# Aaron20127/human-3d-reconstruction

Hardware: AMD Instinct MI355X
Metric: images/sec whole-node, DLA-34+SMPL batch-64 512x512; top-k index bit-match (higher is better)
Workload: dtype bf16; 1 GPU; DLA-34+DCNv2 multi_pose + pose/shape heads -> sigmoid/NMS/top-100 decode -> SMPL 6890-vert LBS; 512x512, batch 64 per GPU (BASELINE configs[2]); batch_per_gpu=64, global_batch=64, K=100, smpl_people_per_image=100, parallelism=dp1 (image shards, one all-gather of dets), collective=none (one rank), steps_in_flight=3, hip_graph=False, dcn_margin=auto, images=64 distinct synthetic images (h3d_amd.synth.synth_image_batch, seed 317), weights=synthetic (h3d_amd.synth, seed 0, gain 1.25, offset_scale 0.5)

## Files before the change

### human-3d-reconstruction_amd/_lib.py

```python
import ctypes
import os

_HERE = os.path.dirname(os.path.abspath(__file__))
LIB_PATH = os.path.join(_HERE, "csrc", "libh3d_hip.so")

H3D_F32, H3D_BF16, H3D_F16, H3D_F16X3 = 0, 1, 2, 3
OP_STEM, OP_CONV, OP_DCN, OP_MAXPOOL, OP_UPADD, OP_COPY, OP_HEADS, OP_DCN_V1, OP_DCN_FUSED = 1, 2, 3, 4, 5, 6, 7, 8, 9
OP_CONV_STREAM, OP_DCN_FUSED_F16, OP_DCN_FUSED_STREAM, OP_STEM3, OP_UPDCN_F16 = 10, 11, 12, 13, 14
OP_IM2COL, OP_MAXPOOL3, OP_DEPTH2SPACE = 15, 16, 17
HEADS_MAX = 16
OUT_NHWC, OUT_NCHW_F32, OUT_NHWC_F32, OUT_NHWC_F16 = 0, 1, 2, 3
DCN_INPUT_NHWC, DCN_OUTPUT_NHWC, DCN_F32_MFMA = 1, 2, 4
ABI_VERSION = 4

DCN_AUX_BYTES = 256
DCN_FUSED_BIAS_WMAX, DCN_FUSED_BIAS_AMAX = 32, 34
OPF_DCN_MASK_FINAL, OPF_DCN_RAW_PACK, OPF_DCN_ACT_MAXIMA, TUNE_DCN_ABLATE_MASK = 0x800, 0x100000, 0x200000, 0x1f
OPF_DCN_FUSED_RAW_PACK, OPF_DCN_FUSED_SCALED_INPUT = 0x100000, 0x200000
TUNE_DCN_FUSED_X3_MARGIN2, TUNE_DCN_FUSED_X3_MARGIN6, TUNE_DCN_FUSED_X3_MARGIN4, TUNE_DCN_FUSED_X3_ABLATE_MASK = 0x2000, 0x4000, 0x8000, 0x1f
OPF_DCN_STREAM_NO_SLOTS, OPF_DCN_STREAM_WIDE_MARGIN, OPF_DCN_STREAM_SLOTS512, OPF_DCN_STREAM_F16_INPUT = 0x1000, 0x8000, 0x10000, 0x40000
OPF_DCN_STREAM_STATS, OPF_DCN_STREAM_VARIANT_MASK = 0x20000, 0x58600
TUNE_DCN_STREAM_FORCE_NARROW_WG, TUNE_DCN_STREAM_FORCE_WIDE_WG = 0x200, 0x400
TUNE_DCN_STREAM_F16_DCN5, TUNE_DCN_STREAM_F16_KEEP_DCN3, TUNE_DCN_STREAM_ABLATE_MASK = 0x4000, 0x2000, 0x1f
TUNE_DCN_STREAM_X3_MARGIN2, TUNE_DCN_STREAM_X3_MARGIN3, TUNE_DCN_STREAM_X3_MARGIN4, TUNE_DCN_STREAM_X3_ABLATE_MASK = 0x4000, 0x8000, 0x10000, 0x1f
TUNE_DCN_F16_ONE_WG_PER_CU, TUNE_DCN_F16_ABLATE_MASK = 0x100, 0xff
TUNE_CONV_STREAM_TILE_MASK, TUNE_CONV_STREAM_AUTO, TUNE_CONV_STREAM_ROUND4_RULE, TUNE_CONV_STREAM_ABLATE_MASK = 0xffff, 1, 0x10000000, 0x1f0000
TUNE_CONV_TILE, TUNE_CONV_HALO_TILE, TUNE_CONV_FORCE_GEMM, TUNE_CONV_GEMM_TILE_MASK = 0x1000, 0x2000, 0x4000, 0xf00
TUNE_CONV_X3_TILED, TUNE_CONV_X3_TILE_MASK, TUNE_CONV_X3_CK16, TUNE_CONV_X3_MT2 = 0x1000, 0x1fff, 0x2000, 0x4000
TUNE_UPADD_TAPS_GLOBAL, TUNE_UPADD_TAPS_LDS, OPF_UPADD_FOLDED = 1, 2, 0x100
TUNE_HEADS_SEPARATE_BIAS, TUNE_HEADS_ABLATE_MASK = 0x200, 0xff
TUNE_HEADS_SPARSE_LDS_PATCH, TUNE_HEADS_SPARSE_WAVES4 = 0x400, 0x800


def TUNE_DCN_STREAM_DCN5_XP(xp):
    return xp << 16


def TUNE_DCN_STREAM_DCN5_XP_OF(reserved):
    return (reserved >> 16) & 0xff


def TUNE_CONV_STREAM_TILE(variant, mt, waves):
    return variant << 12 | mt << 8 | waves

# ... 234 lines not shown
```

### human-3d-reconstruction_amd/csrc/conv2.hip

```cpp
#include "common.h"
#include "epilogue.h"

struct Conv2Args {
    const char *in;
    const char *wimg;
    const float *bias;
    const char *res;
    char *out;
    int B, H, W, Cin, in_cs;
    int Ho, Wo, Cout, out_cs, res_cs, relu, out_mode;
    int G, tiles_x, tiles_y;
    int dbg;
    int xcd;
    int f16;
    unsigned long long *stamps;
};

template <int MT, int WAVES, int S = 1, int SLOTS = 2, int NT = 1>
struct Conv2Cfg {
    static constexpr int TH = 2 * WAVES * NT;
    static constexpr int HROWS = (TH - 1) * S + 3;
    static constexpr int HCOLS = 15 * S + 3;
    static constexpr int PPR = S;
    static constexpr int ROWB = PPR * 1024;
    static constexpr int ROWS = HROWS * PPR;
    static constexpr int HALO = ROWS * 1024;
    static constexpr int WROW = 19 * 16;
    static constexpr int WGRP = 32 * WROW;
    static constexpr int WPIECES = (MT * WGRP + 1023) / 1024;
    static constexpr int WALLOC = WPIECES * 1024;
    static constexpr int SLOT = HALO + WALLOC;
    static constexpr int LDS_EPI = WAVES * ((NT * 32 * (64 * MT + 16) + 1023) / 1024 * 1024);
    static constexpr int LDS_RING = SLOTS * SLOT;
    static constexpr int LDS = LDS_RING > LDS_EPI ? LDS_RING : LDS_EPI;
    static constexpr int THREADS = 64 * WAVES;
    static constexpr int HP = (ROWS + WAVES - 1) / WAVES;
    static constexpr int WP = (WPIECES + WAVES - 1) / WAVES;
};

typedef __attribute__((address_space(3))) void lds_void;

template <int MT, int WAVES, int S, int NT>
__device__ __forceinline__ void conv2_issue(const char *in_b, int in_bytes, const char *wimg, int w_bytes, char *base,
                                            const int *hoff, int woff, int wv, int s, int wsrc, int dbg = 0)
{
    using C = Conv2Cfg<MT, WAVES, S, 2, NT>;
    const auto r_in = __builtin_amdgcn_make_buffer_rsrc((void *)in_b, 0, in_bytes, 0x00020000);
    const auto r_w = __builtin_amdgcn_make_buffer_rsrc((void *)wimg, 0, w_bytes, 0x00020000);
#pragma unroll
    for (int j = 0; j < C::HP; ++j) {
        const int p = wv + j * WAVES;
        if (p < C::ROWS && !(dbg & 8)) __builtin_amdgcn_raw_ptr_buffer_load_lds(r_in, (lds_void *)(base + p * 1024), 16, hoff[j], s * 32, 0, 0);
    }
#pragma unroll
    for (int j = 0; j < C::WP; ++j) {
        const int p = wv + j * WAVES;
        if (p < C::WPIECES && !(dbg & 16))
            __builtin_amdgcn_raw_ptr_buffer_load_lds(r_w, (lds_void *)(base + C::HALO + p * 1024), 16, woff, wsrc + p * 1024, 0, 0);
    }
}

template <typename T, int MT, int WAVES, int EPI, int S = 1, int SLOTS = 2, int NT = 1, bool PIPE = false>
__global__ __launch_bounds__(64 * WAVES) void conv2_kernel(Conv2Args a)
{
    using C = Conv2Cfg<MT, WAVES, S, SLOTS, NT>;
    using E = ET<T>;
    static_assert(sizeof(T) == 2, "2-byte element types");
    __shared__ __attribute__((aligned(1024))) char smem[C::LDS];

    const int tid = threadIdx.x;
    const int l = tid & 63, r = l & 31, h = l >> 5;
    const int wv = __builtin_amdgcn_readfirstlane(tid >> 6);
    const int tiles = a.tiles_x * a.tiles_y;
    const int bid = h3d_tile_id(blockIdx.x, gridDim.x, a.xcd);
    const int b = bid / tiles;
    const int t = bid - b * tiles;
    const int ty = t / a.tiles_x, tx = t - ty * a.tiles_x;
    const int oy0 = ty * C::TH, ox0 = tx * 16;
    const int g0 = blockIdx.y * MT;
    const int cout0 = g0 * 32;
    const int nst = a.Cin >> 4;

// ... 12 lines not shown
    }
    const int woff = l * 16;

    const int py = 2 * NT * wv + (r >> 4), px = r & 15;
    const int boff = py * S * C::ROWB + px * S * 48 + h * 16;
    const int aoff = C::HALO + r * C::WROW + h * 16;

    f32x16 acc[MT][NT];
#pragma unroll
    for (int m = 0; m < MT; ++m)
#pragma unroll
        for (int n = 0; n < NT; ++n)
#pragma unroll
            for (int i = 0; i < 16; ++i) acc[m][n][i] = 0.f;

    constexpr int AHEAD = SLOTS > 1 ? SLOTS - 1 : 1;
    constexpr int PMIN = C::ROWS / WAVES + C::WPIECES / WAVES;
    static_assert(AHEAD <= 2 && PMIN <= 63, "counted vmcnt wait");
    constexpr int WAIT_PMIN = 0x0f70 | (PMIN & 15) | ((PMIN >> 4) << 14);
#pragma unroll
    for (int j = 0; j < AHEAD; ++j)
        if (j < nst && (SLOTS > 1 || j == 0))
            conv2_issue<MT, WAVES, S, NT>(in_b, (int)img_bytes, a.wimg, w_bytes, smem + j * C::SLOT, hoff, woff, wv, j, (j * a.G + g0) * C::WGRP, H3D_DBG(a));
    int cslot = 0, pslot = AHEAD % SLOTS;
#ifdef H3D_ABLATE
    unsigned long long t_bar = 0, t_iss = 0;
    const unsigned long long t_start = __builtin_readcyclecounter();
#endif
    for (int s = 0; s < nst; ++s) {
        if constexpr (SLOTS == 1) {
            if (s > 0) {
                __syncthreads();
                conv2_issue<MT, WAVES, S, NT>(in_b, (int)img_bytes, a.wimg, w_bytes, smem, hoff, woff, wv, s, (s * a.G + g0) * C::WGRP, H3D_DBG(a));
            }
        }
        if (AHEAD == 2 && s + 1 < nst) __builtin_amdgcn_s_waitcnt(WAIT_PMIN);
        else __builtin_amdgcn_s_waitcnt(0x0f70);
#ifdef H3D_ABLATE
        const unsigned long long tb0 = __builtin_readcyclecounter();
#endif
        h3d_barrier_keep_vmcnt();
#ifdef H3D_ABLATE
        const unsigned long long tb1 = __builtin_readcyclecounter();
        t_bar += tb1 - tb0;
#endif
        if (SLOTS > 1 && s + AHEAD < nst && !(H3D_DBG(a) & 1))
            conv2_issue<MT, WAVES, S, NT>(in_b, (int)img_bytes, a.wimg, w_bytes, smem + pslot * C::SLOT, hoff, woff, wv, s + AHEAD, ((s + AHEAD) * a.G + g0) * C::WGRP, H3D_DBG(a));
#ifdef H3D_ABLATE
        t_iss += __builtin_readcyclecounter() - tb1;
#endif
        const char *sl = smem + cslot * C::SLOT;
        cslot = cslot + 1 == SLOTS ? 0 : cslot + 1;
        pslot = pslot + 1 == SLOTS ? 0 : pslot + 1;
        if (H3D_DBG(a) & 2) continue;
        if constexpr (PIPE) {
            typename E::frag fb[2][NT], fa[2][MT];
            auto rd = [&](int tap, int q) {
                const int dy = tap / 3, dx = tap - 3 * dy;
#pragma unroll
                for (int n = 0; n < NT; ++n) fb[q][n] = E::lds_frag(sl + boff + (2 * n * S + dy) * C::ROWB + dx * 48);
#pragma unroll
                for (int m = 0; m < MT; ++m) fa[q][m] = E::lds_frag(sl + aoff + m * C::WGRP + tap * 32);
            };
            rd(0, 0);
            __builtin_amdgcn_sched_group_barrier(0x100, MT + NT, 0);
#pragma unroll
            for (int tap = 0; tap < 9; ++tap) {
                if (tap + 1 < 9) rd(tap + 1, (tap + 1) & 1);
#pragma unroll
                for (int m = 0; m < MT; ++m)
#pragma unroll
                    for (int n = 0; n < NT; ++n) E::mma(acc[m][n], fa[tap & 1][m], fb[tap & 1][n]);
                if (tap + 1 < 9) __builtin_amdgcn_sched_group_barrier(0x100, MT + NT, 0);
                __builtin_amdgcn_sched_group_barrier(0x008, MT * NT, 0);
            }
        } else {
#pragma unroll
        for (int tap = 0; tap < 9; ++tap) {
            const int dy = tap / 3, dx = tap - 3 * dy;
            typename E::frag fb[NT];
#pragma unroll
            for (int n = 0; n < NT; ++n) fb[n] = E::lds_frag(sl + boff + (2 * n * S + dy) * C::ROWB + dx * 48);
            typename E::frag fa[MT];
#pragma unroll
            for (int m = 0; m < MT; ++m) fa[m] = E::lds_frag(sl + aoff + m * C::WGRP + tap * 32);
#pragma unroll
            for (int m = 0; m < MT; ++m)
#pragma unroll
                for (int n = 0; n < NT; ++n) E::mma(acc[m][n], fa[m], fb[n]);
        }
        }
    }

#ifdef H3D_ABLATE
    if (a.stamps && blockIdx.x < 65536 && blockIdx.y == 0 && l == 0) {
        const unsigned long long t_loop = __builtin_readcyclecounter() - t_start;
        if (wv < 4) a.stamps[blockIdx.x * H3D_NSTAMP + wv] = t_bar;
        if (wv >= WAVES - 3) a.stamps[blockIdx.x * H3D_NSTAMP + 4 + (wv - (WAVES - 3))] = t_bar;
        if (wv == 0) a.stamps[blockIdx.x * H3D_NSTAMP + 7] = (t_iss << 32) | (t_loop & 0xffffffffull);
    }
#endif
    EpiArgs e;
    e.bias = a.bias; e.res = a.res; e.out = a.out; e.Ho = a.Ho; e.Wo = a.Wo; e.Cout = a.Cout;
    e.out_cs = a.out_cs; e.res_cs = a.res_cs; e.relu = a.relu; e.out_mode = a.out_mode;
    if constexpr (EPI == 2) {
        __syncthreads();
        tile_epilogue_lds<T, MT, NT>(acc, e, b, oy0, ox0, cout0, wv, l, smem + wv * epi_lds_stride<MT, NT>());
    } else {
        tile_epilogue<T, MT, NT, EPI == 1>(acc, e, b, oy0, ox0, cout0, wv, r, h);
    }
}

template <int MT, int WAVES, int S = 1, int SLOTS = 2, int NT = 1, bool PIPE = false>
static int launch_conv2_cfg(const Conv2Args &a0, hipStream_t st)
{
    using C = Conv2Cfg<MT, WAVES, S, SLOTS, NT>;
    static_assert(C::LDS <= 160 * 1024, "LDS budget");
    Conv2Args a = a0;
    a.tiles_x = cdiv(a.Wo, 16);
    a.tiles_y = cdiv(a.Ho, C::TH);
    a.xcd = h3d_xcd_mode();
#ifdef H3D_ABLATE
    a.stamps = h3d_stamp_buffer();
#else
    a.stamps = nullptr;
#endif
    dim3 grid(a.B * a.tiles_x * a.tiles_y, cdiv(cdiv(a.Cout, 32), MT));
    const bool lean = a.out_mode == H3D_OUT_NHWC && a.Cout % 4 == 0 && ((uintptr_t)a.bias & 15) == 0;
    const int epi = (MT >= 2 && lean && a.Cout % 8 == 0 && a.out_cs % 8 == 0 && ((uintptr_t)a.out & 15) == 0 && !(a.dbg & 4)) ? 2 : lean ? 1 : 0;
    return h3d_by_values([&](auto f16, auto e) {
        using T = std::conditional_t<f16, f16_t, bf16_t>;
        constexpr bool pipe = PIPE && e == 2;
        return h3d_launch({"conv2_kernel", h3d_tag<T>{}, MT, WAVES, e, S, SLOTS, NT, h3d_opt(pipe)},
                          conv2_kernel<T, MT, WAVES, e, S, SLOTS, NT, pipe>, grid, dim3(C::THREADS), 0, st, a);
    }, h3d_vals<false, true>{}, a.f16 != 0, h3d_vals<0, 1, 2>{}, epi);
}

int h3d_launch_conv_stream(const h3d_op &op, hipStream_t st)
{
    if (!op.in || !op.w || !op.bias || !op.out) H3D_FAIL(H3D_ERR_ARG, "conv_stream: null pointer");
    if (op.dtype != H3D_BF16 && op.dtype != H3D_F16) H3D_FAIL(H3D_ERR_DTYPE, "conv_stream: bf16 / fp16 plans only (dtype %d)", op.dtype);
    if (op.ksize != 3 || (op.stride != 1 && op.stride != 2) || op.Ho != (op.H - 1) / op.stride + 1 || op.Wo != (op.W - 1) / op.stride + 1)
        H3D_FAIL(H3D_ERR_UNSUPPORTED, "conv_stream: covers 3x3 p1 with stride 1 or 2 (k=%d s=%d, %dx%d -> %dx%d)", op.ksize, op.stride,
                 op.H, op.W, op.Ho, op.Wo);
    if (op.Cin % 16 || op.in_cs % 8 || op.Cin > op.in_cs)
        H3D_FAIL(H3D_ERR_SHAPE, "conv_stream: Cin=%d (stride %d) must be a multiple of 16", op.Cin, op.in_cs);
    if ((size_t)op.H * op.W * op.in_cs * 2 >= 0x7ffffff0ull) H3D_FAIL(H3D_ERR_SHAPE, "conv_stream: image of 2 GiB or more");
    if (op.wrows % 128 || op.wrows < op.Cout)
        H3D_FAIL(H3D_ERR_SHAPE, "conv_stream: packed weight/bias rows %d for Cout %d (Cout padded to 128 expected)", op.wrows, op.Cout);
    if (op.out_mode != H3D_OUT_NCHW_F32 && (op.out_cs % 4 || op.Cout > op.out_cs))
        H3D_FAIL(H3D_ERR_SHAPE, "conv_stream: out channel stride %d", op.out_cs);
    if (op.in2 && (op.in2_cs % 4 || op.Cout > op.in2_cs)) H3D_FAIL(H3D_ERR_SHAPE, "conv_stream: residual stride %d", op.in2_cs);
    Conv2Args a;
    a.in = (const char *)op.in; a.wimg = (const char *)op.w; a.bias = op.bias; a.res = (const char *)op.in2;
    a.out = (char *)op.out; a.B = op.B; a.H = op.H; a.W = op.W; a.Cin = op.Cin; a.in_cs = op.in_cs;
    a.Ho = op.Ho; a.Wo = op.Wo; a.Cout = op.Cout; a.out_cs = op.out_cs; a.res_cs = op.in2_cs; a.relu = op.relu; a.out_mode = op.out_mode;
    a.G = op.wrows / 32; a.tiles_x = a.tiles_y = 0;
    a.f16 = op.dtype == H3D_F16;
    a.dbg = H3D_TUNE_CONV_STREAM_ABLATE_OF(op.reserved);
    const int tile = op.reserved & H3D_TUNE_CONV_STREAM_TILE_MASK;
    const int gq = cdiv(op.Cout, 32);
    auto nblk = [&](int th, int mt) { return (long)op.B * cdiv(op.Wo, 16) * cdiv(op.Ho, th) * cdiv(gq, mt); };
    if (op.stride == 2) {
        switch (tile) {
        case H3D_TUNE_CONV_STREAM_TILE(4, 4, 4): return launch_conv2_cfg<4, 4, 2, 1>(a, st);
        case H3D_TUNE_CONV_STREAM_TILE(4, 4, 8): return launch_conv2_cfg<4, 8, 2, 1>(a, st);
        case H3D_TUNE_CONV_STREAM_TILE(4, 2, 4): return launch_conv2_cfg<2, 4, 2, 1>(a, st);
        default: break;
        }
        if (gq >= 4) return tile == H3D_TUNE_CONV_STREAM_TILE(2, 4, 4) ? launch_conv2_cfg<4, 4, 2>(a, st) : launch_conv2_cfg<4, 4, 2, 1>(a, st);
        if (gq >= 2) return launch_conv2_cfg<2, 4, 2>(a, st);
        return launch_conv2_cfg<1, 4, 2>(a, st);
    }
    if (tile) {
// ... 43 lines not shown
```

### human-3d-reconstruction_amd/csrc/ops.hip

```cpp
#include "common.h"
#include <stdlib.h>

static thread_local char g_err[512] = "";

void h3d_set_error(const char *fmt, ...)
{
    va_list ap;
    va_start(ap, fmt);
    vsnprintf(g_err, sizeof(g_err), fmt, ap);
    va_end(ap);
}

static thread_local char g_kname[160] = "";
static thread_local bool g_dry = false;

bool h3d_note_kernel(const char *fmt, ...)
{
    va_list ap;
    va_start(ap, fmt);
    vsnprintf(g_kname, sizeof(g_kname), fmt, ap);
    va_end(ap);
    return g_dry;
}

// ... 26 lines not shown
#ifdef H3D_ABLATE
    f |= H3D_BUILD_ABLATE;
#endif
    return f;
}

int h3d_launch_conv(const h3d_op &op, hipStream_t st);
int h3d_launch_stem(const h3d_op &op, hipStream_t st);
int h3d_launch_elementwise(const h3d_op &op, hipStream_t st);
int h3d_launch_dcn(const h3d_op &op, hipStream_t st);
int h3d_launch_heads(const h3d_op &op, hipStream_t st);
int h3d_launch_dcn2(const h3d_op &op, hipStream_t st);
int h3d_launch_dcn3(const h3d_op &op, hipStream_t st);
int h3d_launch_dcn3_fold(const h3d_op &op, const h3d_op &up, hipStream_t st, bool *folded);
int h3d_launch_conv_stream(const h3d_op &op, hipStream_t st);
int h3d_launch_dcn4(const h3d_op &op, hipStream_t st);
int h3d_launch_updcn(const h3d_op &op, hipStream_t st);
int h3d_launch_stem3(const h3d_op &op, hipStream_t st);
int h3d_launch_extra(const h3d_op &op, hipStream_t st);

static int run_one(const h3d_op &op, int i, hipStream_t st, const h3d_op *up = nullptr, bool *folded = nullptr);

static int run_at(const h3d_op *ops, int i, int n, hipStream_t st, bool *folded)
{
    *folded = false;
    if (i + 1 < n && ops[i].kind == H3D_OP_DCN_FUSED_STREAM && ops[i + 1].kind == H3D_OP_UPADD && (ops[i + 1].reserved & H3D_OPF_UPADD_FOLDED) &&
        ops[i].out && ops[i + 1].in2 == ops[i].out)
        return run_one(ops[i], i, st, &ops[i + 1], folded);
    return run_one(ops[i], i, st);
}

extern "C" int h3d_op_kernel_name(const h3d_op *op, char *buf, int buflen)
{
    if (!op || !buf || buflen <= 0) H3D_FAIL(H3D_ERR_ARG, "op_kernel_name: null argument");
    g_dry = true;
    g_kname[0] = 0;
    const int rc = run_one(*op, 0, nullptr);
    g_dry = false;
    snprintf(buf, buflen, "%s", g_kname);
    return rc;
}

extern "C" int h3d_run_ops_timed(const h3d_op *ops, int n, void *stream, float *ms)
{
    if (!ops || n <= 0 || !ms) H3D_FAIL(H3D_ERR_ARG, "run_ops_timed: null argument");
    hipStream_t st = (hipStream_t)stream;
    hipEvent_t *ev = (hipEvent_t *)malloc(sizeof(hipEvent_t) * (n + 1));
    if (!ev) H3D_FAIL(H3D_ERR_ARG, "run_ops_timed: out of host memory");
    for (int i = 0; i <= n; ++i) (void)hipEventCreate(&ev[i]);
    int rc = H3D_OK;
    (void)hipEventRecord(ev[0], st);
    for (int i = 0; i < n; ++i) ms[i] = 0.f;
    for (int i = 0; i < n && rc == H3D_OK; ++i) {
        bool folded = false;
        rc = run_at(ops, i, n, st, &folded);
        (void)hipEventRecord(ev[i + 1], st);
        if (folded) {
            ++i;
            ms[i] = -1.f;
            (void)hipEventRecord(ev[i + 1], st);
        }
    }
    if (rc == H3D_OK) {
        (void)hipEventSynchronize(ev[n]);
        for (int i = 0; i < n; ++i) {
            if (ms[i] < 0.f) ms[i] = 0.f;
            else (void)hipEventElapsedTime(&ms[i], ev[i], ev[i + 1]);
        }
    }
    for (int i = 0; i <= n; ++i) (void)hipEventDestroy(ev[i]);
    free(ev);
    return rc;
}

extern "C" int h3d_run_ops(const h3d_op *ops, int n, void *stream)
{
    if (!ops || n < 0) H3D_FAIL(H3D_ERR_ARG, "run_ops: null plan");
    hipStream_t st = (hipStream_t)stream;
    for (int i = 0; i < n; ++i) {
        bool folded = false;
        const int rc = run_at(ops, i, n, st, &folded);
        if (rc != H3D_OK) return rc;
        if (folded) ++i;
    }
    return H3D_OK;
}

static int run_one(const h3d_op &op, int i, hipStream_t st, const h3d_op *up, bool *folded)
{
    int rc;
    if (op.B <= 0 || op.H <= 0 || op.W <= 0 || op.Ho <= 0 || op.Wo <= 0 || op.Cin <= 0 || op.Cout <= 0) {
        h3d_set_error("op %d (kind %d): non-positive dimension", i, op.kind);
        return H3D_ERR_SHAPE;
    }
    switch (op.kind) {
    case H3D_OP_STEM: rc = h3d_launch_stem(op, st); break;
    case H3D_OP_STEM3: rc = h3d_launch_stem3(op, st); break;
    case H3D_OP_CONV: rc = h3d_launch_conv(op, st); break;
// ... 9 lines not shown
    case H3D_OP_UPDCN_F16:
        h3d_set_error("op %d (kind %d): a superseded kernel generation, built only by `make EXTRA=1` (csrc/Makefile)", i, op.kind);
        return H3D_ERR_UNSUPPORTED;
#endif
    case H3D_OP_DCN_FUSED:
    case H3D_OP_DCN_FUSED_STREAM: rc = up ? h3d_launch_dcn3_fold(op, *up, st, folded) : h3d_launch_dcn3(op, st); break;
    case H3D_OP_HEADS: rc = h3d_launch_heads(op, st); break;
    case H3D_OP_MAXPOOL:
    case H3D_OP_UPADD:
    case H3D_OP_COPY: rc = h3d_launch_elementwise(op, st); break;
    case H3D_OP_IM2COL:
    case H3D_OP_MAXPOOL3:
    case H3D_OP_DEPTH2SPACE: rc = h3d_launch_extra(op, st); break;
    default: h3d_set_error("op %d: unknown kind %d", i, op.kind); return H3D_ERR_ARG;
    }
    if (rc != H3D_OK) {
        char tmp[400];
        snprintf(tmp, sizeof(tmp), "%s", h3d_last_error());
        h3d_set_error("op %d (kind %d): %s", i, op.kind, tmp);
    }
    return rc;
}
```

### human-3d-reconstruction_amd/detector.py

```python
import torch

from . import _lib, decode, smpl as _smpl
from .model import create_model
from .utils import _transpose_and_gather_feat

MULTI_POSE_HEADS = {"hm": 1, "wh": 2, "hps": 34, "reg": 2, "hm_hp": 17, "hp_offset": 2}
CTDET_HEADS = {"hm": 80, "wh": 2, "reg": 2}
SMPL_HEADS = {"pose": 72, "shape": 10}
WHOLE_MAP_HEADS = ("hm", "hm_hp", "hp_offset")
PEAK_HEADS = ("hp_offset",)


class LazyHeads(dict):

    def __init__(self, maps, completer):
        super().__init__(maps)
        self._completer = completer

    @property
    def complete(self):
        return self._completer is None

    def rearm(self, completer):
        self._completer = completer
# ... 84 lines not shown
        if opt.task != "multi_pose":
            raise ValueError("task not defined!")
        self.opt = opt
        self.device = torch.device(device)
        self.model = create_model(opt.arch, opt.heads, opt.head_conv, opt.not_use_dcn, dtype=opt.dtype)
        if state_dict is not None:
            self.model.load_state_dict(state_dict, strict=True)
        self.model.to(self.device).eval()
        self.smpl_model = smpl_model
        self.fused_tail = True
        self.sparse_heads = True
        if opt.arch.replace("-", "_") in ("dla_34", "dla34") and opt.dtype in ("bf16", "f16"):
            self.model.engine_flags["split_heads"] = tuple(h for h in opt.heads if h in WHOLE_MAP_HEADS)
            self.model.engine_flags["peak_heads"] = tuple(h for h in opt.heads if h in PEAK_HEADS)
            self.model.engine_flags["fold_upadd"] = True
        if opt.smpl and smpl_model is None:
            self.smpl_model = _smpl.SMPLModel.synthetic()

    @torch.no_grad()
    def run(self, images, meta=None, slot=0, graph=False):
        if graph and meta is None:
            return self._run_graph(images, slot)
        opt = self.opt
        plan = None
        if self.sparse_heads and not opt.flip_test and images.is_cuda and not self.model.training:
            plan = self.model.engine(images.device).forward_eager(images, slot)
        if plan is not None:
            out = plan.outputs
            top = decode._multi_pose_topk(out["hm"], out.get("hm_hp") if opt.hm_hp else None, opt.K, logits=True)
            if plan.sparse_masks[1] and top["hm_inds"] is not None:
# ... 219 lines not shown
```

### human-3d-reconstruction_amd/plan.py

```python
import ctypes

import torch

from . import _lib, arch, arch_hg, arch_res
from ._lib import H3dOp
from .weights import _TORCH_DT, LOWP

_H3D_DT = {"bf16": _lib.H3D_BF16, "f16": _lib.H3D_F16, "f32": _lib.H3D_F32, "f16x3": _lib.H3D_F16X3}
DCN_F16IN = _lib.OPF_DCN_STREAM_F16_INPUT


class View:
    __slots__ = ("buf", "H", "W", "C", "cs", "coff", "es")

    def __init__(self, buf, H, W, C, cs, coff, es):
        self.buf, self.H, self.W, self.C, self.cs, self.coff, self.es = buf, H, W, C, cs, coff, es

    @property
    def ptr(self):
        return self.buf.data_ptr() + self.coff * self.es

    def slice(self, c0, c):
        assert c0 + c <= self.C
        return View(self.buf, self.H, self.W, c, self.cs, self.coff + c0, self.es)
# ... 15 lines not shown
        fuse_upnode_min_f=2,
        dcn_slots512=0,
        dcn_wide_margin=0,
        node_f16=True,
        share_pool=True,
        fuse_stem=True,
        fuse_stem_proj=False,
        mixed_heads=0,
        wide_heads_m2=0,
        x3_dcn_patches=True,
        stem_s2_direct=True,
        conv1x1_th16_min_cin=0,
        lower_heads=True,
        split_heads=(),
        fold_upadd=False,
        peak_heads=(),
    )

    def __init__(self, pw, B, H, W, **flags):
        unknown = set(flags) - set(self.FLAGS)
        if unknown:
            raise TypeError("unknown lowering flags: %s" % sorted(unknown))
        for k, v in self.FLAGS.items():
            setattr(self, k, flags.get(k, v))
        self.stream_s2_min_cin = 64
        if pw.arch == "hourglass" and (H % 128 or W % 128):
            raise RuntimeError("Hourglass-104: input height/width must be multiples of 128 (got %dx%d): the published test "
                               "code pads to (x|127)+1" % (H, W))
        if H % 32 or W % 32:
            raise RuntimeError("input height/width must be multiples of 32 (got %dx%d): the reference pads "
# ... 38 lines not shown
        op.kind, op.dtype, op.B = kind, _H3D_DT[self.dtype], self.B
        if x is not None:
            op.in_, op.H, op.W, op.Cin, op.in_cs = x.ptr, x.H, x.W, x.C, x.cs
        if out is not None:
            op.out, op.Ho, op.Wo, op.Cout, op.out_cs = out.ptr, out.H, out.W, out.C, out.cs
        if x2 is not None:
            op.in2, op.in2_cs = x2.ptr, x2.cs
        for k, v in kw.items():
            setattr(op, k, v)
        if not emit:
            return op
        self.ops.append(op)
        return len(self.ops) - 1

    def conv(self, x, wkey, out=None, bkey=None, bn=None, stride=1, relu=True, res=None, out_mode=_lib.OUT_NHWC,
             pad_cout_to=None):
        wshape = self.pw.sd[wkey].shape
        if (self.stream_convs and self.pw.dtype in LOWP and wshape[2] == 3 and wshape[1] % 16 == 0
                and (stride == 1 or (stride == 2 and wshape[1] >= self.stream_s2_min_cin and self.stream_s2))
                and out_mode == _lib.OUT_NHWC and pad_cout_to is None):
            return self._conv_stream(x, wkey, out, bkey, bn, relu, res, stride)
        wp, bp, cout, cin, k, rows = self.pw.conv(wkey, bkey, bn, pad_cout_to)
        assert cin == x.C, (wkey, cin, x.C)
        Ho = (x.H + 2 * (k // 2) - k) // stride + 1
        Wo = (x.W + 2 * (k // 2) - k) // stride + 1
        if out_mode == _lib.OUT_NHWC_F32:
            out = self._alloc(Ho, Wo, cout, torch.float32)
        elif out is None:
            out = self._alloc(Ho, Wo, cout)
        assert (out.H, out.W, out.C) == (Ho, Wo, cout), (wkey, out.H, out.W, out.C, Ho, Wo, cout)
        tune = 0
        if (k == 1 and stride == 1 and self.conv1x1_th16_min_cin and cin >= self.conv1x1_th16_min_cin and cin % 64 == 0
                and cout > 32 and self.pw.dtype in LOWP):
            tune = _lib.TUNE_CONV_1X1_TILE(4 if cout > 64 else 2, 16)
        self._op(_lib.OP_CONV, x, out, res, w=wp.data_ptr(), bias=bp.data_ptr(), ksize=k, stride=stride, relu=int(relu),
                 out_mode=out_mode, wrows=rows, reserved=tune, wexp=self.pw.wexp.get(wp.data_ptr(), 0))
        return out

    def _conv_stream(self, x, wkey, out, bkey, bn, relu, res, stride=1):
        wimg, bp, cout, cin, rows = self.pw.conv_stream(wkey, bkey, bn)
        assert cin == x.C, (wkey, cin, x.C)
        Ho, Wo = (x.H - 1) // stride + 1, (x.W - 1) // stride + 1
        if out is None:
            out = self._alloc(Ho, Wo, cout)
        assert (out.H, out.W, out.C) == (Ho, Wo, cout), (wkey, out.H, out.W, out.C)
        self._op(_lib.OP_CONV_STREAM, x, out, res, w=wimg.data_ptr(), bias=bp.data_ptr(), ksize=3, stride=stride, relu=int(relu),
                 out_mode=_lib.OUT_NHWC, wrows=rows)
        return out

    def dcn(self, x, om, wkey, bkey, bn):
        wp, bp, cout, cin, k, rows = self.pw.conv(wkey, bkey, bn, as_half=True)
        assert cin == x.C and k == 3
        out = self._alloc(x.H, x.W, cout)
        self._op(_lib.OP_DCN, x, out, om, w=wp.data_ptr(), bias=bp.data_ptr(), ksize=3, stride=1, relu=1, out_mode=_lib.OUT_NHWC,
                 wrows=rows)
        return out

    def pool(self, x, out=None):
        if out is None:
            out = self._alloc(x.H // 2, x.W // 2, x.C)
        assert out.C == x.C
        self._op(_lib.OP_MAXPOOL, x, out, ksize=2, stride=2)
        return out

    def upadd(self, x, skip, wkey, f16=False, private_skip=False):
        w, k = self.pw.up(wkey)
        f = k // 2
        out = self._alloc(x.H * f, x.W * f, x.C)
        assert (skip.H, skip.W, skip.C) == (out.H, out.W, out.C), wkey
        fold = (private_skip and self.ops and self.ops[-1].kind == _lib.OP_DCN_FUSED_STREAM and self.ops[-1].out == skip.ptr
                and (skip.coff, skip.cs) == (0, skip.C))
        self._op(_lib.OP_UPADD, x, out, skip, w=w.data_ptr(), ksize=k, stride=f, out_mode=_lib.OUT_NHWC_F16 if f16 else _lib.OUT_NHWC,
                 reserved=_lib.OPF_UPADD_FOLDED if fold else 0)
        return out

    def _block(self, x, p, stride, residual, out):
        t = self.conv(x, p + ".conv1.weight", bn=p + ".bn1", stride=stride)
        return self.conv(t, p + ".conv2.weight", bn=p + ".bn2", res=residual, out=out)

    def _tree1(self, x, p, cin, cout, stride, level_root, out, cat=None, bottom=None, residual=None):
        Ho, Wo = x.H // stride, x.W // stride
        if cat is None:
            cat = self._alloc(Ho, Wo, 2 * cout + (cin if level_root else 0))
        s_x2, s_x1 = cat.slice(0, cout), cat.slice(cout, cout)
        if residual is not None:
            assert stride > 1 and not level_root and cin != cout and (residual.H, residual.W, residual.C) == (Ho, Wo, cout)
        elif bottom is not None:
            assert stride > 1 and not level_root and (bottom.H, bottom.W, bottom.C) == (Ho, Wo, cin)
        elif stride > 1:
            bottom = self.pool(x, cat.slice(2 * cout, cin) if level_root else None)
        else:
            bottom = x
        if residual is not None:
            pass
        elif cin != cout:
            residual = self.conv(bottom, p + ".project.0.weight", bn=p + ".project.1", relu=False)
        else:
            residual = bottom
        self._block(x, p + ".tree1", stride, residual, s_x1)
        self._block(s_x1, p + ".tree2", 1, s_x1, s_x2)
        return self.conv(cat, p + ".root.conv.weight", bn=p + ".root.bn", out=out)

    def _tree2(self, x, p, cin, cout, out):
        Ho, Wo = x.H // 2, x.W // 2
        cat = self._alloc(Ho, Wo, 2 * cout + cin + cout)
        pooled = self.pool(x, cat.slice(2 * cout, cin))
        x1 = self._tree1(x, p + ".tree1", cin, cout, 2, False, cat.slice(2 * cout + cin, cout),
                         bottom=pooled if self.share_pool else None)
        return self._tree1(x1, p + ".tree2", cout, cout, 1, False, out, cat=cat)

    def _dcn_f16_ok(self, p):
        w = self.pw.sd[p + ".conv.weight"]
        return (self.pw.use_dcn and self.fuse_offsets and self.stream_dcn and self.pw.dtype == "bf16"
                and w.shape[1] == 64 and w.shape[0] <= 64)

    def _node_f16_ok(self, p):
# ... 297 lines not shown
```

### include/h3d.h

```cpp
#ifndef H3D_H
#define H3D_H

#include <stddef.h>
#include <stdint.h>

#ifdef __cplusplus
extern "C" {
#endif

#define H3D_OK 0
#define H3D_ERR_SHAPE (-1)
#define H3D_ERR_DTYPE (-2)
#define H3D_ERR_LAUNCH (-3)
#define H3D_ERR_UNSUPPORTED (-4)
#define H3D_ERR_ARG (-5)

#define H3D_F32 0
#define H3D_BF16 1
#define H3D_F16 2
#define H3D_F16X3 3

const char *h3d_last_error(void);
int h3d_abi_version(void);
#define H3D_ABI_VERSION 4
// ... 196 lines not shown
#define H3D_TUNE_CONV_X3_TILE(mt, waves, th) (H3D_TUNE_CONV_X3_TILED | (mt) << 8 | (waves) << 4 | (th) >> 3)
enum {
    H3D_TUNE_CONV_X3_TILED = 0x1000,
    H3D_TUNE_CONV_X3_TILE_MASK = 0x1fff,
    H3D_TUNE_CONV_X3_CK16 = 0x2000,
    H3D_TUNE_CONV_X3_MT2 = 0x4000
};

enum {
    H3D_TUNE_UPADD_TAPS_GLOBAL = 1,
    H3D_TUNE_UPADD_TAPS_LDS = 2,
    H3D_OPF_UPADD_FOLDED = 0x100
};

enum {
    H3D_TUNE_HEADS_SEPARATE_BIAS = 0x200,
    H3D_TUNE_HEADS_SPARSE_LDS_PATCH = 0x400,
    H3D_TUNE_HEADS_SPARSE_WAVES4 = 0x800,
    H3D_TUNE_HEADS_ABLATE_MASK = 0xff
};

int h3d_dcn_fused_ck(int Cin, int Cout);

int h3d_dcn_far_samples(const h3d_op *op, int32_t *per_tile, void *stream);

int h3d_run_ops(const h3d_op *ops, int n, void *stream);

int h3d_run_ops_timed(const h3d_op *ops, int n, void *stream, float *ms);
int h3d_op_kernel_name(const h3d_op *op, char *buf, int buflen);

// ... 247 lines not shown
```

Baseline: 10820 images/s.

## Fuse tree-entry maxpool and 1x1 projection into stride-2 streamed conv kernel

At DLA tree entries, the 2x2 maxpool, the 1x1 project conv and the stride-2 3x3 conv1 all read the same input. This change folds all three into one streamed conv kernel. The pool is computed from the centre taps already loaded into the halo, and the projection is a second MFMA accumulator fed by projection filters staged in LDS. The plan flags the triple of ops and the runner dispatches the fused launch. This removes two launches and the extra global reads and writes of the pooled tensor. In exchange the kernel uses more LDS and registers, is forced to one slot, and routes some narrow-Cin stride-2 convs through the stream path.

```diff
diff --git a/human-3d-reconstruction_amd/_lib.py b/human-3d-reconstruction_amd/_lib.py
--- a/human-3d-reconstruction_amd/_lib.py
+++ b/human-3d-reconstruction_amd/_lib.py
@@ -28,6 +28,7 @@
 TUNE_CONV_TILE, TUNE_CONV_HALO_TILE, TUNE_CONV_FORCE_GEMM, TUNE_CONV_GEMM_TILE_MASK = 0x1000, 0x2000, 0x4000, 0xf00
 TUNE_CONV_X3_TILED, TUNE_CONV_X3_TILE_MASK, TUNE_CONV_X3_CK16, TUNE_CONV_X3_MT2 = 0x1000, 0x1fff, 0x2000, 0x4000
 TUNE_UPADD_TAPS_GLOBAL, TUNE_UPADD_TAPS_LDS, OPF_UPADD_FOLDED = 1, 2, 0x100
+OPF_TREE_ENTRY, OPF_TREE_ENTRY_PRIVATE_POOL = 0x20000000, 0x40000000
 TUNE_HEADS_SEPARATE_BIAS, TUNE_HEADS_ABLATE_MASK = 0x200, 0xff
 TUNE_HEADS_SPARSE_LDS_PATCH, TUNE_HEADS_SPARSE_WAVES4 = 0x400, 0x800
 
diff --git a/human-3d-reconstruction_amd/csrc/conv2.hip b/human-3d-reconstruction_amd/csrc/conv2.hip
--- a/human-3d-reconstruction_amd/csrc/conv2.hip
+++ b/human-3d-reconstruction_amd/csrc/conv2.hip
@@ -13,10 +13,15 @@
     int dbg;
     int xcd;
     int f16;
+    const char *pw;
+    const float *pbias;
+    char *pout;
+    char *pool_out;
+    int pwrows, pout_cs, pool_cs;
     unsigned long long *stamps;
 };
 
-template <int MT, int WAVES, int S = 1, int SLOTS = 2, int NT = 1>
+template <int MT, int WAVES, int S = 1, int SLOTS = 2, int NT = 1, bool ENTRY = false>
 struct Conv2Cfg {
     static constexpr int TH = 2 * WAVES * NT;
     static constexpr int HROWS = (TH - 1) * S + 3;
@@ -29,7 +34,8 @@
     static constexpr int WGRP = 32 * WROW;
     static constexpr int WPIECES = (MT * WGRP + 1023) / 1024;
     static constexpr int WALLOC = WPIECES * 1024;
-    static constexpr int SLOT = HALO + WALLOC;
+    static constexpr int PALLOC = ENTRY ? MT * 1024 : 0;
+    static constexpr int SLOT = HALO + WALLOC + PALLOC;
     static constexpr int LDS_EPI = WAVES * ((NT * 32 * (64 * MT + 16) + 1023) / 1024 * 1024);
     static constexpr int LDS_RING = SLOTS * SLOT;
     static constexpr int LDS = LDS_RING > LDS_EPI ? LDS_RING : LDS_EPI;
@@ -60,12 +66,22 @@
     }
 }
 
-template <typename T, int MT, int WAVES, int EPI, int S = 1, int SLOTS = 2, int NT = 1, bool PIPE = false>
-__global__ __launch_bounds__(64 * WAVES) void conv2_kernel(Conv2Args a)
-{
-    using C = Conv2Cfg<MT, WAVES, S, SLOTS, NT>;
+template <int MT, int WAVES>
+__device__ __forceinline__ void conv2_issue_proj(const char *pw, int pw_bytes, char *base, int poff, int wv, int s, int mstep)
+{
+    const auto r_p = __builtin_amdgcn_make_buffer_rsrc((void *)pw, 0, pw_bytes, 0x00020000);
+#pragma unroll
+    for (int m = 0; m < MT; ++m)
+        if (m % WAVES == wv) __builtin_amdgcn_raw_ptr_buffer_load_lds(r_p, (lds_void *)(base + m * 1024), 16, poff, m * mstep + s * 32, 0, 0);
+}
+
+template <typename T, int MT, int WAVES, int EPI, int S = 1, int SLOTS = 2, int NT = 1, bool PIPE = false, bool ENTRY = false>
+__global__ __launch_bounds__(64 * WAVES, ENTRY ? 2 : 1) void conv2_kernel(Conv2Args a)
+{
+    using C = Conv2Cfg<MT, WAVES, S, SLOTS, NT, ENTRY>;
     using E = ET<T>;
     static_assert(sizeof(T) == 2, "2-byte element types");
+    static_assert(!ENTRY || (S == 2 && NT == 1 && EPI == 2 && !PIPE && SLOTS == 1 && MT <= WAVES), "ENTRY: the one-slot stride-2 tiles with the LDS-transposed epilogue");
     __shared__ __attribute__((aligned(1024))) char smem[C::LDS];
 
     const int tid = threadIdx.x;
@@ -108,6 +124,20 @@
 #pragma unroll
             for (int i = 0; i < 16; ++i) acc[m][n][i] = 0.f;
 
+    [[maybe_unused]] f32x16 acc2[ENTRY ? MT : 1][1];
+    [[maybe_unused]] const int poff = ((cout0 + (l >> 1)) * a.Cin + (l & 1) * 8) * 2;
+    [[maybe_unused]] const int pw_bytes = a.pwrows * a.Cin * 2;
+    if constexpr (ENTRY) {
+#pragma unroll
+        for (int m = 0; m < MT; ++m)
+#pragma unroll
+            for (int i = 0; i < 16; ++i) acc2[m][0][i] = 0.f;
+    }
+    auto issue = [&](char *base, int s) {
+        conv2_issue<MT, WAVES, S, NT>(in_b, (int)img_bytes, a.wimg, w_bytes, base, hoff, woff, wv, s, (s * a.G + g0) * C::WGRP, H3D_DBG(a));
+        if constexpr (ENTRY) conv2_issue_proj<MT, WAVES>(a.pw, pw_bytes, base + C::HALO + C::WALLOC, poff, wv, s, 32 * a.Cin * 2);
+    };
+
     constexpr int AHEAD = SLOTS > 1 ? SLOTS - 1 : 1;
     constexpr int PMIN = C::ROWS / WAVES + C::WPIECES / WAVES;
     static_assert(AHEAD <= 2 && PMIN <= 63, "counted vmcnt wait");
@@ -115,7 +145,7 @@
 #pragma unroll
     for (int j = 0; j < AHEAD; ++j)
         if (j < nst && (SLOTS > 1 || j == 0))
-            conv2_issue<MT, WAVES, S, NT>(in_b, (int)img_bytes, a.wimg, w_bytes, smem + j * C::SLOT, hoff, woff, wv, j, (j * a.G + g0) * C::WGRP, H3D_DBG(a));
+            issue(smem + j * C::SLOT, j);
     int cslot = 0, pslot = AHEAD % SLOTS;
 #ifdef H3D_ABLATE
     unsigned long long t_bar = 0, t_iss = 0;
@@ -125,7 +155,7 @@
         if constexpr (SLOTS == 1) {
             if (s > 0) {
                 __syncthreads();
-                conv2_issue<MT, WAVES, S, NT>(in_b, (int)img_bytes, a.wimg, w_bytes, smem, hoff, woff, wv, s, (s * a.G + g0) * C::WGRP, H3D_DBG(a));
+                issue(smem, s);
             }
         }
         if (AHEAD == 2 && s + 1 < nst) __builtin_amdgcn_s_waitcnt(WAIT_PMIN);
@@ -139,7 +169,7 @@
         t_bar += tb1 - tb0;
 #endif
         if (SLOTS > 1 && s + AHEAD < nst && !(H3D_DBG(a) & 1))
-            conv2_issue<MT, WAVES, S, NT>(in_b, (int)img_bytes, a.wimg, w_bytes, smem + pslot * C::SLOT, hoff, woff, wv, s + AHEAD, ((s + AHEAD) * a.G + g0) * C::WGRP, H3D_DBG(a));
+            issue(smem + pslot * C::SLOT, s + AHEAD);
 #ifdef H3D_ABLATE
         t_iss += __builtin_readcyclecounter() - tb1;
 #endif
@@ -169,6 +199,7 @@
                 __builtin_amdgcn_sched_group_barrier(0x008, MT * NT, 0);
             }
         } else {
+        [[maybe_unused]] float pm[8];
 #pragma unroll
         for (int tap = 0; tap < 9; ++tap) {
             const int dy = tap / 3, dx = tap - 3 * dy;
@@ -182,6 +213,25 @@
             for (int m = 0; m < MT; ++m)
 #pragma unroll
                 for (int n = 0; n < NT; ++n) E::mma(acc[m][n], fa[m], fb[n]);
+            if constexpr (ENTRY) {
+                if (tap == 4) {
+                    unpack16<T>(fb[0].v, pm);
+                } else if (tap == 5 || tap == 7 || tap == 8) {
+                    float x[8];
+                    unpack16<T>(fb[0].v, x);
+#pragma unroll
+                    for (int k = 0; k < 8; ++k) pm[k] = fmaxf(pm[k], x[k]);
+                }
+            }
+        }
+        if constexpr (ENTRY) {
+            typename E::frag pb;
+            pb.v = pack16<T>(pm);
+#pragma unroll
+            for (int m = 0; m < MT; ++m) E::mma(acc2[m][0], E::lds_frag(sl + C::HALO + C::WALLOC + m * 1024 + r * 32 + h * 16), pb);
+            const int oy = oy0 + py, ox = ox0 + px;
+            if (a.pool_out && blockIdx.y == 0 && oy < a.Ho && ox < a.Wo)
+                *reinterpret_cast<u32x4 *>(a.pool_out + ((((size_t)b * a.Ho + oy) * a.Wo + ox) * a.pool_cs + 16 * s + 8 * h) * 2) = pb.v;
         }
         }
     }
@@ -200,6 +250,10 @@
     if constexpr (EPI == 2) {
         __syncthreads();
         tile_epilogue_lds<T, MT, NT>(acc, e, b, oy0, ox0, cout0, wv, l, smem + wv * epi_lds_stride<MT, NT>());
+        if constexpr (ENTRY) {
+            e.bias = a.pbias; e.res = nullptr; e.out = a.pout; e.out_cs = a.pout_cs; e.res_cs = 0; e.relu = 0;
+            tile_epilogue_lds<T, MT, 1>(acc2, e, b, oy0, ox0, cout0, wv, l, smem + wv * epi_lds_stride<MT, NT>());
+        }
     } else {
         tile_epilogue<T, MT, NT, EPI == 1>(acc, e, b, oy0, ox0, cout0, wv, r, h);
     }
@@ -230,7 +284,26 @@
     }, h3d_vals<false, true>{}, a.f16 != 0, h3d_vals<0, 1, 2>{}, epi);
 }
 
-int h3d_launch_conv_stream(const h3d_op &op, hipStream_t st)
+template <int MT>
+static int launch_conv2_entry(const Conv2Args &a0, hipStream_t st)
+{
+    constexpr int WAVES = 4, S = 2, SLOTS = 1;
+    using C = Conv2Cfg<MT, WAVES, S, SLOTS, 1, true>;
+    static_assert(2 * C::LDS <= 160 * 1024, "LDS budget: two workgroups per CU, as without the project filters");
+    Conv2Args a = a0;
+    a.tiles_x = cdiv(a.Wo, 16);
+    a.tiles_y = cdiv(a.Ho, C::TH);
+    a.xcd = h3d_xcd_mode();
+    a.stamps = nullptr;
+    dim3 grid(a.B * a.tiles_x * a.tiles_y, cdiv(cdiv(a.Cout, 32), MT));
+    return h3d_by_values([&](auto f16) {
+        using T = std::conditional_t<f16, f16_t, bf16_t>;
+        return h3d_launch({"conv2_kernel", h3d_tag<T>{}, MT, WAVES, 2, S, SLOTS, 1, false, true},
+                          conv2_kernel<T, MT, WAVES, 2, S, SLOTS, 1, false, true>, grid, dim3(C::THREADS), 0, st, a);
+    }, h3d_vals<false, true>{}, a.f16 != 0);
+}
+
+static int conv_stream_check(const h3d_op &op)
 {
     if (!op.in || !op.w || !op.bias || !op.out) H3D_FAIL(H3D_ERR_ARG, "conv_stream: null pointer");
     if (op.dtype != H3D_BF16 && op.dtype != H3D_F16) H3D_FAIL(H3D_ERR_DTYPE, "conv_stream: bf16 / fp16 plans only (dtype %d)", op.dtype);
@@ -245,6 +318,11 @@
     if (op.out_mode != H3D_OUT_NCHW_F32 && (op.out_cs % 4 || op.Cout > op.out_cs))
         H3D_FAIL(H3D_ERR_SHAPE, "conv_stream: out channel stride %d", op.out_cs);
     if (op.in2 && (op.in2_cs % 4 || op.Cout > op.in2_cs)) H3D_FAIL(H3D_ERR_SHAPE, "conv_stream: residual stride %d", op.in2_cs);
+    return H3D_OK;
+}
+
+static Conv2Args conv_stream_args(const h3d_op &op)
+{
     Conv2Args a;
     a.in = (const char *)op.in; a.wimg = (const char *)op.w; a.bias = op.bias; a.res = (const char *)op.in2;
     a.out = (char *)op.out; a.B = op.B; a.H = op.H; a.W = op.W; a.Cin = op.Cin; a.in_cs = op.in_cs;
@@ -252,6 +330,49 @@
     a.G = op.wrows / 32; a.tiles_x = a.tiles_y = 0;
     a.f16 = op.dtype == H3D_F16;
     a.dbg = H3D_TUNE_CONV_STREAM_ABLATE_OF(op.reserved);
+    a.pw = nullptr; a.pbias = nullptr; a.pout = nullptr; a.pool_out = nullptr; a.pwrows = a.pout_cs = a.pool_cs = 0;
+    return a;
+}
+
+bool h3d_conv_stream_entry_takes(const h3d_op &pool, const h3d_op &proj, const h3d_op &conv)
+{
+    if (pool.kind != H3D_OP_MAXPOOL || proj.kind != H3D_OP_CONV || conv.kind != H3D_OP_CONV_STREAM) return false;
+    if (!(pool.reserved & H3D_OPF_TREE_ENTRY) || !(proj.reserved & H3D_OPF_TREE_ENTRY) || !(conv.reserved & H3D_OPF_TREE_ENTRY)) return false;
+    const int gq = cdiv(conv.Cout, 32);
+    if ((conv.reserved & ~H3D_OPF_TREE_ENTRY) != (gq >= 4 ? 0 : H3D_TUNE_CONV_STREAM_TILE(4, 2, 4))) return false;
+    if ((proj.reserved & ~H3D_OPF_TREE_ENTRY) || (pool.reserved & ~(H3D_OPF_TREE_ENTRY | H3D_OPF_TREE_ENTRY_PRIVATE_POOL))) return false;
+    if ((conv.dtype != H3D_BF16 && conv.dtype != H3D_F16) || pool.dtype != conv.dtype || proj.dtype != conv.dtype) return false;
+    if (!pool.in || !pool.out || !proj.w || !proj.bias || !proj.out || proj.in2) return false;
+    if (proj.in != pool.out || proj.in_cs != pool.out_cs || conv.in != pool.in || conv.in_cs != pool.in_cs) return false;
+    const int B = conv.B, H = conv.H, W = conv.W, C = conv.Cin;
+    if (B <= 0 || H <= 0 || W <= 0 || C <= 0 || conv.Cout <= 0) return false;
+    if (pool.B != B || proj.B != B || pool.H != H || pool.W != W || (H & 1) || (W & 1)) return false;
+    if (pool.Cin != C || pool.Cout != C || proj.Cin != C || C > pool.out_cs) return false;
+    const int Ho = H / 2, Wo = W / 2;
+    if (conv.ksize != 3 || conv.stride != 2 || conv.Ho != Ho || conv.Wo != Wo || pool.Ho != Ho || pool.Wo != Wo) return false;
+    if (proj.ksize != 1 || proj.stride != 1 || proj.H != Ho || proj.W != Wo || proj.Ho != Ho || proj.Wo != Wo) return false;
+    if (proj.Cout != conv.Cout || proj.relu || proj.wexp || proj.out_mode != H3D_OUT_NHWC || conv.out_mode != H3D_OUT_NHWC) return false;
+    if (conv.Cout % 8 || gq < 2 || proj.wrows < cdiv(conv.Cout, 128) * 128 || (long long)proj.wrows * C * 2 >= 0x7ffffff0ll) return false;
+    if (conv.out_cs % 8 || proj.out_cs % 8 || proj.Cout > proj.out_cs || pool.out_cs % 8) return false;
+    if (((uintptr_t)conv.out & 15) || ((uintptr_t)conv.bias & 15) || ((uintptr_t)proj.out & 15) || ((uintptr_t)proj.bias & 15) || ((uintptr_t)proj.w & 15) ||
+        ((uintptr_t)pool.out & 15))
+        return false;
+    return conv_stream_check(conv) == H3D_OK;
+}
+
+int h3d_launch_conv_stream_entry(const h3d_op &pool, const h3d_op &proj, const h3d_op &conv, hipStream_t st)
+{
+    Conv2Args a = conv_stream_args(conv);
+    a.pw = (const char *)proj.w; a.pbias = proj.bias; a.pout = (char *)proj.out; a.pwrows = proj.wrows; a.pout_cs = proj.out_cs;
+    a.pool_out = (pool.reserved & H3D_OPF_TREE_ENTRY_PRIVATE_POOL) ? nullptr : (char *)pool.out;
+    a.pool_cs = pool.out_cs;
+    return cdiv(conv.Cout, 32) >= 4 ? launch_conv2_entry<4>(a, st) : launch_conv2_entry<2>(a, st);
+}
+
+int h3d_launch_conv_stream(const h3d_op &op, hipStream_t st)
+{
+    H3D_TRY(conv_stream_check(op));
+    const Conv2Args a = conv_stream_args(op);
     const int tile = op.reserved & H3D_TUNE_CONV_STREAM_TILE_MASK;
     const int gq = cdiv(op.Cout, 32);
     auto nblk = [&](int th, int mt) { return (long)op.B * cdiv(op.Wo, 16) * cdiv(op.Ho, th) * cdiv(gq, mt); };
diff --git a/human-3d-reconstruction_amd/csrc/ops.hip b/human-3d-reconstruction_amd/csrc/ops.hip
--- a/human-3d-reconstruction_amd/csrc/ops.hip
+++ b/human-3d-reconstruction_amd/csrc/ops.hip
@@ -64,19 +64,31 @@
 int h3d_launch_dcn3(const h3d_op &op, hipStream_t st);
 int h3d_launch_dcn3_fold(const h3d_op &op, const h3d_op &up, hipStream_t st, bool *folded);
 int h3d_launch_conv_stream(const h3d_op &op, hipStream_t st);
+bool h3d_conv_stream_entry_takes(const h3d_op &pool, const h3d_op &proj, const h3d_op &conv);
+int h3d_launch_conv_stream_entry(const h3d_op &pool, const h3d_op &proj, const h3d_op &conv, hipStream_t st);
 int h3d_launch_dcn4(const h3d_op &op, hipStream_t st);
 int h3d_launch_updcn(const h3d_op &op, hipStream_t st);
 int h3d_launch_stem3(const h3d_op &op, hipStream_t st);
 int h3d_launch_extra(const h3d_op &op, hipStream_t st);
 
 static int run_one(const h3d_op &op, int i, hipStream_t st, const h3d_op *up = nullptr, bool *folded = nullptr);
+static int fail_at(int rc, const h3d_op &op, int i);
 
-static int run_at(const h3d_op *ops, int i, int n, hipStream_t st, bool *folded)
+static int run_at(const h3d_op *ops, int i, int n, hipStream_t st, int *folded)
 {
-    *folded = false;
+    *folded = 0;
     if (i + 1 < n && ops[i].kind == H3D_OP_DCN_FUSED_STREAM && ops[i + 1].kind == H3D_OP_UPADD && (ops[i + 1].reserved & H3D_OPF_UPADD_FOLDED) &&
-        ops[i].out && ops[i + 1].in2 == ops[i].out)
-        return run_one(ops[i], i, st, &ops[i + 1], folded);
+        ops[i].out && ops[i + 1].in2 == ops[i].out) {
+        bool pair = false;
+        const int rc = run_one(ops[i], i, st, &ops[i + 1], &pair);
+        *folded = pair;
+        return rc;
+    }
+    if (i + 2 < n && ops[i].kind == H3D_OP_MAXPOOL && (ops[i].reserved & H3D_OPF_TREE_ENTRY) &&
+        h3d_conv_stream_entry_takes(ops[i], ops[i + 1], ops[i + 2])) {
+        *folded = 2;
+        return fail_at(h3d_launch_conv_stream_entry(ops[i], ops[i + 1], ops[i + 2], st), ops[i], i);
+    }
     return run_one(ops[i], i, st);
 }
 
@@ -102,10 +114,10 @@
     (void)hipEventRecord(ev[0], st);
     for (int i = 0; i < n; ++i) ms[i] = 0.f;
     for (int i = 0; i < n && rc == H3D_OK; ++i) {
-        bool folded = false;
+        int folded = 0;
         rc = run_at(ops, i, n, st, &folded);
         (void)hipEventRecord(ev[i + 1], st);
-        if (folded) {
+        for (; folded > 0; --folded) {
             ++i;
             ms[i] = -1.f;
             (void)hipEventRecord(ev[i + 1], st);
@@ -128,10 +140,10 @@
     if (!ops || n < 0) H3D_FAIL(H3D_ERR_ARG, "run_ops: null plan");
     hipStream_t st = (hipStream_t)stream;
     for (int i = 0; i < n; ++i) {
-        bool folded = false;
+        int folded = 0;
         const int rc = run_at(ops, i, n, st, &folded);
         if (rc != H3D_OK) return rc;
-        if (folded) ++i;
+        i += folded;
     }
     return H3D_OK;
 }
@@ -171,6 +183,11 @@
     case H3D_OP_DEPTH2SPACE: rc = h3d_launch_extra(op, st); break;
     default: h3d_set_error("op %d: unknown kind %d", i, op.kind); return H3D_ERR_ARG;
     }
+    return fail_at(rc, op, i);
+}
+
+static int fail_at(int rc, const h3d_op &op, int i)
+{
     if (rc != H3D_OK) {
         char tmp[400];
         snprintf(tmp, sizeof(tmp), "%s", h3d_last_error());
diff --git a/human-3d-reconstruction_amd/detector.py b/human-3d-reconstruction_amd/detector.py
--- a/human-3d-reconstruction_amd/detector.py
+++ b/human-3d-reconstruction_amd/detector.py
@@ -122,6 +122,7 @@
             self.model.engine_flags["split_heads"] = tuple(h for h in opt.heads if h in WHOLE_MAP_HEADS)
             self.model.engine_flags["peak_heads"] = tuple(h for h in opt.heads if h in PEAK_HEADS)
             self.model.engine_flags["fold_upadd"] = True
+            self.model.engine_flags["fold_tree_entry"] = True
         if opt.smpl and smpl_model is None:
             self.smpl_model = _smpl.SMPLModel.synthetic()
 
diff --git a/human-3d-reconstruction_amd/plan.py b/human-3d-reconstruction_amd/plan.py
--- a/human-3d-reconstruction_amd/plan.py
+++ b/human-3d-reconstruction_amd/plan.py
@@ -53,6 +53,7 @@
         lower_heads=True,
         split_heads=(),
         fold_upadd=False,
+        fold_tree_entry=False,
         peak_heads=(),
     )
 
@@ -121,12 +122,13 @@
         return len(self.ops) - 1
 
     def conv(self, x, wkey, out=None, bkey=None, bn=None, stride=1, relu=True, res=None, out_mode=_lib.OUT_NHWC,
-             pad_cout_to=None):
+             pad_cout_to=None, entry=False):
         wshape = self.pw.sd[wkey].shape
         if (self.stream_convs and self.pw.dtype in LOWP and wshape[2] == 3 and wshape[1] % 16 == 0
-                and (stride == 1 or (stride == 2 and wshape[1] >= self.stream_s2_min_cin and self.stream_s2))
+                and (stride == 1 or (stride == 2 and (wshape[1] >= self.stream_s2_min_cin or entry) and self.stream_s2))
                 and out_mode == _lib.OUT_NHWC and pad_cout_to is None):
-            return self._conv_stream(x, wkey, out, bkey, bn, relu, res, stride)
+            tile = _lib.TUNE_CONV_STREAM_TILE(4, 2, 4) if entry and stride == 2 and 64 <= wshape[0] < 128 else 0
+            return self._conv_stream(x, wkey, out, bkey, bn, relu, res, stride, reserved=tile)
         wp, bp, cout, cin, k, rows = self.pw.conv(wkey, bkey, bn, pad_cout_to)
         assert cin == x.C, (wkey, cin, x.C)
         Ho = (x.H + 2 * (k // 2) - k) // stride + 1
@@ -144,7 +146,7 @@
                  out_mode=out_mode, wrows=rows, reserved=tune, wexp=self.pw.wexp.get(wp.data_ptr(), 0))
         return out
 
-    def _conv_stream(self, x, wkey, out, bkey, bn, relu, res, stride=1):
+    def _conv_stream(self, x, wkey, out, bkey, bn, relu, res, stride=1, reserved=0):
         wimg, bp, cout, cin, rows = self.pw.conv_stream(wkey, bkey, bn)
         assert cin == x.C, (wkey, cin, x.C)
         Ho, Wo = (x.H - 1) // stride + 1, (x.W - 1) // stride + 1
@@ -152,7 +154,7 @@
             out = self._alloc(Ho, Wo, cout)
         assert (out.H, out.W, out.C) == (Ho, Wo, cout), (wkey, out.H, out.W, out.C)
         self._op(_lib.OP_CONV_STREAM, x, out, res, w=wimg.data_ptr(), bias=bp.data_ptr(), ksize=3, stride=stride, relu=int(relu),
-                 out_mode=_lib.OUT_NHWC, wrows=rows)
+                 out_mode=_lib.OUT_NHWC, wrows=rows, reserved=reserved)
         return out
 
     def dcn(self, x, om, wkey, bkey, bn):
@@ -181,8 +183,8 @@
                  reserved=_lib.OPF_UPADD_FOLDED if fold else 0)
         return out
 
-    def _block(self, x, p, stride, residual, out):
-        t = self.conv(x, p + ".conv1.weight", bn=p + ".bn1", stride=stride)
+    def _block(self, x, p, stride, residual, out, entry=False):
+        t = self.conv(x, p + ".conv1.weight", bn=p + ".bn1", stride=stride, entry=entry)
         return self.conv(t, p + ".conv2.weight", bn=p + ".bn2", res=residual, out=out)
 
     def _tree1(self, x, p, cin, cout, stride, level_root, out, cat=None, bottom=None, residual=None):
@@ -190,6 +192,8 @@
         if cat is None:
             cat = self._alloc(Ho, Wo, 2 * cout + (cin if level_root else 0))
         s_x2, s_x1 = cat.slice(0, cout), cat.slice(cout, cout)
+        entry = self.fold_tree_entry and self.share_pool and stride == 2 and residual is None and cin != cout
+        private = bottom is None and not level_root
         if residual is not None:
             assert stride > 1 and not level_root and cin != cout and (residual.H, residual.W, residual.C) == (Ho, Wo, cout)
         elif bottom is not None:
@@ -198,15 +202,31 @@
             bottom = self.pool(x, cat.slice(2 * cout, cin) if level_root else None)
         else:
             bottom = x
+        n_proj = len(self.ops)
         if residual is not None:
             pass
         elif cin != cout:
             residual = self.conv(bottom, p + ".project.0.weight", bn=p + ".project.1", relu=False)
         else:
             residual = bottom
-        self._block(x, p + ".tree1", stride, residual, s_x1)
+        self._block(x, p + ".tree1", stride, residual, s_x1, entry=entry)
+        if entry:
+            self._flag_tree_entry(n_proj - 1, private)
         self._block(s_x1, p + ".tree2", 1, s_x1, s_x2)
         return self.conv(cat, p + ".root.conv.weight", bn=p + ".root.bn", out=out)
+
+    def _flag_tree_entry(self, i, private):
+        if i < 0 or i + 3 > len(self.ops):
+            return
+        pool, proj, conv1 = self.ops[i:i + 3]
+        tile = 0 if conv1.Cout >= 128 else _lib.TUNE_CONV_STREAM_TILE(4, 2, 4)
+        if (pool.kind == _lib.OP_MAXPOOL and proj.kind == _lib.OP_CONV and conv1.kind == _lib.OP_CONV_STREAM and proj.ksize == 1 and conv1.stride == 2
+                and (proj.in_, proj.in_cs) == (pool.out, pool.out_cs) and (conv1.in_, conv1.in_cs) == (pool.in_, pool.in_cs)
+                and proj.Cout == conv1.Cout >= 64 and pool.H % 2 == 0 and pool.W % 2 == 0 and conv1.reserved == tile
+                and not (proj.reserved or pool.reserved)):
+            pool.reserved = _lib.OPF_TREE_ENTRY | (_lib.OPF_TREE_ENTRY_PRIVATE_POOL if private else 0)
+            proj.reserved = _lib.OPF_TREE_ENTRY
+            conv1.reserved = tile | _lib.OPF_TREE_ENTRY
 
     def _tree2(self, x, p, cin, cout, out):
         Ho, Wo = x.H // 2, x.W // 2
diff --git a/include/h3d.h b/include/h3d.h
--- a/include/h3d.h
+++ b/include/h3d.h
@@ -234,6 +234,11 @@
 };
 
 enum {
+    H3D_OPF_TREE_ENTRY = 0x20000000,
+    H3D_OPF_TREE_ENTRY_PRIVATE_POOL = 0x40000000
+};
+
+enum {
     H3D_TUNE_HEADS_SEPARATE_BIAS = 0x200,
     H3D_TUNE_HEADS_SPARSE_LDS_PATCH = 0x400,
     H3D_TUNE_HEADS_SPARSE_WAVES4 = 0x800,
```

Result: faster. 10980 images/s, median of 6 (+1.5%).
